# zenghjian/SceneSplat

Measured on AMD Instinct MI355X. Metric: Gaussians/s encoder fwd+bwd, 102k-pt chunks, higher is better.
Workload: dtype bf16

## Files before the change

include/scenesplat_hip.h:

```cpp
#ifndef SCENESPLAT_HIP_H
#define SCENESPLAT_HIP_H
#include <stddef.h>
#include <stdint.h>

#ifdef __cplusplus
extern "C" {
#endif

struct ihipStream_t;
typedef struct ihipStream_t* ss_stream_t;

#define SS_MAX_ORDERS 8
enum { SS_ORDER_Z = 0, SS_ORDER_Z_TRANS = 1, SS_ORDER_HILBERT = 2, SS_ORDER_HILBERT_TRANS = 3 };
enum { SS_DTYPE_F32 = 0, SS_DTYPE_BF16 = 1 };
enum { SS_ATTN_SIMT = 0, SS_ATTN_MFMA = 1 };
enum { SS_OK = 0, SS_ERR_ARG = 1, SS_ERR_LAUNCH = 2, SS_ERR_WORKSPACE = 3 };

int ss_version(void);

int ss_serialize_encode(const int32_t* grid_coord, const int32_t* batch, int64_t n, int depth, const int* orders,
                        int num_orders, int64_t* codes, ss_stream_t stream);
int ss_offsets_to_batch(const int32_t* offsets, int num_batches, int64_t n, int32_t* batch, ss_stream_t stream);
int ss_count_duplicates(const int64_t* sorted_keys, int64_t n, int32_t* count, ss_stream_t stream);
int ss_grid_coord_max(const int32_t* grid_coord, int64_t n, int32_t* out_max, ss_stream_t stream);
// ... 86 lines not shown

int ss_subm_conv_fwd(const void* in, const void* weight, const float* bias, const int32_t* nbr, const int32_t* rowperm,
                     void* out, int64_t n, int cin, int cout, int taps, int out_dtype, ss_stream_t stream);
int ss_subm_weight_mirror(const void* w, void* wt, int cout, int taps, int cin, ss_stream_t stream);
int ss_stream_create_cu_mask(int nwords, const uint32_t* mask, void** stream_out);
int ss_subm_im2col(const void* src, const int32_t* nbr, void* dst, int64_t n, int taps, int64_t row_bytes, ss_stream_t stream);
int ss_gemm8_ok(int64_t m, int k, int n, int taps);
int ss_subm_conv_fwd_pipe(const void* in, const void* weight, const float* bias, const int32_t* nbr, const int32_t* rowperm,
                          void* out, int64_t n, int cin, int cout, int taps, int out_dtype, ss_stream_t stream);
int ss_subm_conv_fwd_pipe_walk(const void* in, const void* weight, const float* bias, const int32_t* nbr_walk, const int32_t* rowperm,
                               void* out, int64_t n, int cin, int cout, int taps, int out_dtype, ss_stream_t stream);
int ss_subm_conv_fwd_uses_pipe(int64_t n, int cin, int cout, int taps);
int ss_subm_conv_fwd_walk(const void* in, const void* weight, const float* bias, const int32_t* nbr, const int32_t* nbr_walk,
                          const int32_t* rowperm, void* out, int64_t n, int cin, int cout, int taps, int out_dtype, ss_stream_t stream);
int ss_linear_fwd(const void* x, const void* weight, const float* bias, void* out, int64_t m, int k, int n, int out_dtype,
                  ss_stream_t stream);
int ss_wgrad_xcd_order(void);
int ss_wgrad_set_xcd_order(int on);
int ss_wgrad8_ok(int64_t n, int cin, int cout, int taps);
int ss_subm_conv_wgrad_pipe(const void* in, const void* dout, const int32_t* nbr, const int32_t* rowperm,
                            const int32_t* blk_count, const int32_t* blk_list, float* dweight, int64_t n, int cin, int cout,
                            int taps, ss_stream_t stream);
int ss_linear_wgrad(const void* x, const void* dy, float* dweight, float* dbias, int64_t m, int k_in, int n_out,
                    ss_stream_t stream);
int ss_linear_wgrad_group_plan(int64_t m, int k_in, int n_out, int64_t* desc_words);
int ss_linear_wgrad_tiles(int k_in, int n_out);
int ss_linear_wgrad_group_plan2(int64_t m, int k_in, int n_out, int launch_tiles, int64_t* desc_words);
int ss_linear_wgrad_group(const int64_t* desc, const int32_t* wg_start, int nprob, int total_workgroups, ss_stream_t stream);
int ss_linear_wgrad_group_plan_capped(int64_t m, int k_in, int n_out, int launch_tiles, int max_workgroups, int64_t* desc_words);
int ss_linear_wgrad_group_capped(const int64_t* desc, const int32_t* wg_start, int nprob, int total_items, int max_workgroups,
                                 ss_stream_t stream);
int ss_subm_conv_splits(int64_t n, int cout, int taps);
int ss_subm_conv_fwd_splitk(const void* in, const void* weight, const float* bias, const int32_t* nbr, const int32_t* rowperm,
                            float* acc32, int64_t n, int cin, int cout, int taps, int splits, ss_stream_t stream);
int ss_subm_block_lists(const int32_t* nbr, const int32_t* rowperm, int64_t n, int taps, int32_t* blk_count,
                        int32_t* blk_list, ss_stream_t stream);
int ss_subm_conv_wgrad(const void* in, const void* dout, const int32_t* nbr, const int32_t* rowperm,
                       const int32_t* blk_count, const int32_t* blk_list, float* dweight, int64_t n, int cin, int cout,
                       int taps, ss_stream_t stream);

int ss_subm_f32_ok(int cin_padded, int cout);
int ss_subm_f32_fwd(const float* in, const float* wq, const float* bias, const int32_t* nbr_walk, const int32_t* rowperm,
                    float* out, int64_t n, int cin_padded, int cout, int taps, ss_stream_t stream);
int ss_subm_f32_dgrad_dup(const float* dout_folded, const float* wq, const int32_t* nbr_walk, const int32_t* rowperm, float* din,
                          int64_t n, int cin_padded, int cout, int taps, ss_stream_t stream);
int ss_subm_f32_wgrad(const float* in, const float* dout, const int32_t* nbr_walk, const int32_t* rowperm,
                      const int32_t* blk_count, const int32_t* blk_list, float* dweight, int64_t n, int cin_padded,
                      int cin, int cout, int taps, ss_stream_t stream);

int ss_subm_conv_wgrad_pipe_walk(const void* in, const void* dout, const int32_t* nbr_walk, const int32_t* rowperm,
                                 const int32_t* blk_count, const int32_t* blk_list, float* dweight, int64_t n, int cin, int cout,
                                 int taps, ss_stream_t stream);
int ss_subm_conv_wgrad_uses_pipe(int64_t n, int cin, int cout, int taps);
int ss_subm_conv_wgrad_walk(const void* in, const void* dout, const int32_t* nbr, const int32_t* nbr_walk, const int32_t* rowperm,
                            const int32_t* blk_count, const int32_t* blk_list, float* dweight, int64_t n, int cin, int cout,
                            int taps, ss_stream_t stream);

int ss_add_layernorm_fwd(const void* x, int x_dtype, const void* y, int y_dtype, const float* rowscale,
                         const float* gamma, const float* beta, float eps, void* xout, int xout_dtype, void* xcopy_bf16,
                         void* h, int h_dtype, float* mean, float* rstd, int64_t n, int channels, ss_stream_t stream);
int ss_ln_add_ln_fwd(const void* x, int x_dtype, const void* t, int t_dtype, const float* gamma0, const float* beta0, float eps0,
                     const float* gamma1, const float* beta1, float eps1, float* xout, void* h, int h_dtype, float* stats,
                     int64_t n, int channels, ss_stream_t stream);
int ss_ln_add_ln_bwd(const float* g_xout, const void* g_h, int g_h_dtype, const float* xout, const void* t, int t_dtype,
                     const float* stats, const float* gamma0, const float* gamma1, void* g_x, int g_x_dtype, void* g_t,
                     int g_t_dtype, float* part, int64_t n, int channels, int nblocks, ss_stream_t stream);
int ss_add_layernorm_bwd_blocks(int64_t n);

int ss_block_tail_rows(void);
int ss_block_tail_bwd_blocks(int64_t n);
int ss_block_tail_fwd(const void* feat, const float* x, const float* rs1, const float* rs2, const void* wp, const void* bp,
                      const void* w1, const void* b1, const void* w2, const void* b2, int bias_dtype, const float* gamma, const float* beta,
                      float eps, float* x_mid, float* mean, float* rstd, void* h2, void* u, void* a, float* x_out,
                      void* xcopy_bf16, int64_t n, int channels, ss_stream_t stream);
int ss_block_tail_bwd(const float* g_xout, const void* g_xcopy_bf16, const float* x_mid, const float* mean, const float* rstd,
                      const void* u, const float* rs1, const float* rs2, const float* gamma, const void* wp_t, const void* w1_t,
                      const void* w2_t, float* g_mid, void* dfeat, void* dy2, void* du, void* dy1, float* part, int64_t n,
                      int channels, int nblocks, ss_stream_t stream);
int ss_group_partial_sums_outputs_per_workgroup(void);
int ss_group_partial_sums(const int64_t* desc, const int32_t* wg_start, int nprob, int total_workgroups, ss_stream_t stream);
int ss_transpose16_group(const int64_t* desc, const int32_t* wg_start, int nprob, int total_workgroups, ss_stream_t stream);
int ss_subm_weight_mirror_group_tile(void);
int ss_subm_weight_mirror_group(const int64_t* desc, const int32_t* wg_start, int nprob, int total_workgroups, ss_stream_t stream);
int ss_add_layernorm_bwd(const void* g_xout, int g_xout_dtype, const void* g_xcopy, int g_xcopy_dtype, const void* g_h,
                         int g_h_dtype, const void* v, int v_dtype, const float* mean, const float* rstd,
                         const float* gamma, const float* rowscale, void* g_x, int g_x_dtype, void* g_y, int g_y_dtype,
                         float* dgamma_part, float* dbeta_part, int64_t n, int channels, int nblocks, ss_stream_t stream);

int ss_col_stats(const void* x, int x_dtype, float* shift_out, float* psum, float* psq, int64_t n, int channels,
                 int nblocks, ss_stream_t stream);
int ss_bn_stats_finish(const float* part, const float* shift, int nblocks, int channels, int64_t n, float momentum, float eps,
                       float* running_mean, float* running_var, int64_t* num_batches, float* mean, float* rstd,
                       ss_stream_t stream);
int ss_bn_bwd_finish(const float* part, int nblocks, int channels, int64_t n, float* sums, float* coef, ss_stream_t stream);
int ss_bn_act_fwd(const void* x, int x_dtype, const float* mean, const float* rstd, const float* gamma, const float* beta,
                  int act, void* y, int y_dtype, int64_t n, int channels, ss_stream_t stream);
int ss_bn_act_bwd_reduce(const void* dy, int dy_dtype, const void* x, int x_dtype, const float* mean, const float* rstd,
                         const float* gamma, const float* beta, int act, float* pdz, float* pdzx, int64_t n, int channels,
                         int nblocks, ss_stream_t stream);
int ss_bn_act_bwd_apply(const void* dy, int dy_dtype, const void* x, int x_dtype, const float* mean, const float* rstd,
                        const float* gamma, const float* beta, int act, const float* c1, const float* c2, void* dx,
                        int dx_dtype, int64_t n, int channels, ss_stream_t stream);

int ss_feat_text_scan(const void* feat_bf16, const void* text_bf16, int64_t n, int dim, int num_classes, float* max_prob,
                      int32_t* argmax, const int32_t* idx, float* pred_accum, ss_stream_t stream);

// ... 208 lines not shown
```

scenesplat_amd/csrc/wgrad8.hip:

```cpp
#include "grouped.h"
#include <stdlib.h>

typedef __attribute__((ext_vector_type(8))) __bf16 w8_bf8_t;
typedef __attribute__((ext_vector_type(4))) short w8_s4_t;
typedef __attribute__((ext_vector_type(8))) short w8_s8_t;
typedef __attribute__((address_space(3))) w8_s4_t w8_lds_s4_t;
#define W8_MFMA(a, b, c) __builtin_amdgcn_mfma_f32_16x16x32_bf16((a), (b), (c), 0, 0, 0)

#define W8_BUF 65536
#define W8_HALF 16384
#define W8_OFF_B 32768
#define W8_CHUNK 60
#define W8_OFF_ISITE 131072
#define W8_OFF_JSITE (W8_OFF_ISITE + W8_CHUNK * 64 * 4)
#define W8_LDS_BYTES (W8_OFF_JSITE + W8_CHUNK * 64 * 4)
#define W8_ZERO_ELEMS 4096

__device__ uint4 w8_zero[W8_ZERO_ELEMS / 8];

__device__ __forceinline__ void w8_glds16(const void* gsrc, unsigned lds_wave_base) {
  asm volatile("s_mov_b32 m0, %1\n\ts_nop 0\n\tglobal_load_lds_dwordx4 %0, off" ::"v"(gsrc), "s"(lds_wave_base) : "memory");
}
__device__ __forceinline__ w8_bf8_t w8_tr2(const char* p) {
  w8_s4_t lo = __builtin_amdgcn_ds_read_tr16_b64_v4i16((w8_lds_s4_t*)(p));
// ... 255 lines not shown
  const int row = 8 * W8_XG, full = nb / row * row;
  if (L >= full) return L;
  const int xcd = L & 7, slot = L >> 3;
  return ((slot / W8_XG) * 8 + xcd) * W8_XG + slot % W8_XG;
}

template <bool GATHER>
__global__ void __launch_bounds__(512)
k_wgrad8(const unsigned short* __restrict__ X, const unsigned short* __restrict__ DY, const int32_t* __restrict__ nbr,
         const int32_t* __restrict__ rowperm, const int32_t* __restrict__ blk_count, const int32_t* __restrict__ blk_list,
         float* __restrict__ dW, float* __restrict__ dbias, int n, int Cin, int Cout, int taps, int ntn, int nblocks_total,
         int min_per, int ntiles, int nshares, int walk) {
  int L = (int)blockIdx.x;
  if (walk & 2) L = w8_xcd_order(L, (int)gridDim.x);
  w8_body<GATHER>(X, DY, nbr, rowperm, blk_count, blk_list, dW, dbias, n, Cin, Cout, taps, ntn, nblocks_total, min_per, ntiles,
                  nshares, L, walk & 1);
}

__global__ void __launch_bounds__(512)
k_wgrad8_group(const int64_t* __restrict__ desc, const int32_t* __restrict__ wg_start, int nprob, int nprob_flags) {
  const int b = blockIdx.x;
  const int p = group_owner(wg_start, nprob, b);
  const int64_t* d = desc + (int64_t)p * 8;
  const int64_t m = d[4];
  const uint64_t w5 = (uint64_t)d[5], w6 = (uint64_t)d[6], w7 = (uint64_t)d[7];
  const int k_in = (int)(w5 & 0xffffffffu), n_out = (int)(w5 >> 32);
  const int ntn = (int)(w6 & 0xffffffffu), ntiles = (int)(w6 >> 32);
  const int nshares = (int)(w7 & 0xffffffffu), min_per = (int)(w7 >> 32);
  int L = b - wg_start[p];
  if (nprob_flags & 1) {
    const int a = (8 - (wg_start[p] & 7)) & 7;
    if (L >= a) L = a + w8_xcd_order(L - a, nshares * ntiles - a);
  }
  w8_body<false>((const unsigned short*)d[0], (const unsigned short*)d[1], nullptr, nullptr, nullptr, nullptr, (float*)d[2],
                 (float*)d[3], (int)m, k_in, n_out, 1, ntn, (int)((m + 63) / 64), min_per, ntiles, nshares, L);
}

__global__ void __launch_bounds__(512)
k_wgrad8_group_capped(const int64_t* __restrict__ desc, const int32_t* __restrict__ wg_start, int nprob, int total_items) {
  for (int b = blockIdx.x; b < total_items; b += (int)gridDim.x) {
    const int p = group_owner(wg_start, nprob, b);
    const int64_t* d = desc + (int64_t)p * 8;
    const int64_t m = d[4];
    const uint64_t w5 = (uint64_t)d[5], w6 = (uint64_t)d[6], w7 = (uint64_t)d[7];
    const int k_in = (int)(w5 & 0xffffffffu), n_out = (int)(w5 >> 32);
    const int ntn = (int)(w6 & 0xffffffffu), ntiles = (int)(w6 >> 32);
    const int nshares = (int)(w7 & 0xffffffffu), min_per = (int)(w7 >> 32);
    w8_body<false>((const unsigned short*)d[0], (const unsigned short*)d[1], nullptr, nullptr, nullptr, nullptr, (float*)d[2],
                   (float*)d[3], (int)m, k_in, n_out, 1, ntn, (int)((m + 63) / 64), min_per, ntiles, nshares, b - wg_start[p]);
    __syncthreads();
  }
}

static int w8_xcd_flag = -1;
extern "C" int ss_wgrad_xcd_order(void) {
  if (w8_xcd_flag < 0) { const char* e = getenv("SS_WGRAD_XCD_TRIPLE"); w8_xcd_flag = (e && atoi(e) == 1) ? 1 : 0; }
  return w8_xcd_flag;
}
extern "C" int ss_wgrad_set_xcd_order(int on) { w8_xcd_flag = on ? 1 : 0; return SS_OK; }

extern "C" int ss_wgrad8_ok(int64_t n, int cin, int cout, int taps) {
  return n > 0 && n < (1LL << 31) && cin >= 8 && (cin & 7) == 0 && cin <= W8_ZERO_ELEMS && cout >= 8 && (cout & 7) == 0 &&
         cout <= W8_ZERO_ELEMS && taps >= 1;
}

static int w8_min_per(int64_t busy_tiles, int64_t est_blocks) {
  int64_t per = busy_tiles * est_blocks / 200;
  if (per < 8) per = 8;
  if (per > 160) per = 160;
  return (int)per;
}

static int w8_conv_launch(const void* in, const void* dout, const int32_t* nbr, const int32_t* rowperm, const int32_t* blk_count,
                          const int32_t* blk_list, float* dweight, int64_t n, int cin, int cout, int taps, int walk, hipStream_t stream);

extern "C" int ss_subm_conv_wgrad_pipe(const void* in, const void* dout, const int32_t* nbr, const int32_t* rowperm,
                                       const int32_t* blk_count, const int32_t* blk_list, float* dweight, int64_t n,
                                       int cin, int cout, int taps, hipStream_t stream) {
  return w8_conv_launch(in, dout, nbr, rowperm, blk_count, blk_list, dweight, n, cin, cout, taps, 0, stream);
}
extern "C" int ss_subm_conv_wgrad_pipe_walk(const void* in, const void* dout, const int32_t* nbr_walk, const int32_t* rowperm,
                                            const int32_t* blk_count, const int32_t* blk_list, float* dweight, int64_t n,
                                            int cin, int cout, int taps, hipStream_t stream) {
  return w8_conv_launch(in, dout, nbr_walk, rowperm, blk_count, blk_list, dweight, n, cin, cout, taps, 1, stream);
}

static int w8_conv_launch(const void* in, const void* dout, const int32_t* nbr, const int32_t* rowperm, const int32_t* blk_count,
                          const int32_t* blk_list, float* dweight, int64_t n, int cin, int cout, int taps, int walk, hipStream_t stream) {
  if (n == 0) return SS_OK;
  if (!ss_wgrad8_ok(n, cin, cout, taps) || !blk_count || !blk_list || !nbr) return SS_ERR_ARG;
  const int nblocks = ss_div_up(n, 64);
  const int tm = ss_div_up(cout, 256), tn = ss_div_up(cin, 256);
  static int env_per = -2;
  if (env_per == -2) { const char* e = getenv("SS_WGRAD_MINPER"); env_per = e ? atoi(e) : -1; }
  int min_per = env_per > 0 ? env_per : w8_min_per((int64_t)tm * tn * ((taps + 2) / 3), (int64_t)nblocks * 7 / 10);
  int splits = ss_div_up(nblocks, min_per);
  if (ss_wgrad_xcd_order()) walk |= 2;
  dim3 g((unsigned)((int64_t)taps * splits * tm * tn));
  SS_LAUNCH((k_wgrad8<true>), g, dim3(512), 0, stream, (const unsigned short*)in, (const unsigned short*)dout, nbr, rowperm,
            blk_count, blk_list, dweight, (float*)nullptr, (int)n, cin, cout, taps, tn, nblocks, min_per, tm * tn, splits, walk);
  return SS_OK;
}

static void w8_linear_plan(int64_t m, int k_in, int n_out, int* tm_, int* tn_, int* min_per_, int* splits_, int launch_tiles = 0) {
  const int nblocks = ss_div_up(m, 64);
  const int tm = ss_div_up(n_out, 256), tn = ss_div_up(k_in, 256);
  static int env_per = -2;
  if (env_per == -2) { const char* e = getenv("SS_WGRAD_MINPER"); env_per = e ? atoi(e) : -1; }
  static const int cus = [] {
    int dev = 0, n = 256;
    if (hipGetDevice(&dev) == hipSuccess) (void)hipDeviceGetAttribute(&n, hipDeviceAttributeMultiprocessorCount, dev);
    return n > 0 ? n : 256;
  }();
  const int tiles_all = launch_tiles > tm * tn ? launch_tiles : tm * tn;
  const int shares = cus / tiles_all > 0 ? cus / tiles_all : 1;
  int min_per = env_per > 0 ? env_per : (int)((nblocks + shares - 1) / shares);
  if (env_per <= 0 && min_per < 8) min_per = 8;
  if (min_per > nblocks) min_per = nblocks;
  *tm_ = tm; *tn_ = tn; *min_per_ = min_per; *splits_ = ss_div_up(nblocks, min_per);
}

extern "C" int ss_linear_wgrad_tiles(int k_in, int n_out) { return ss_div_up(n_out, 256) * ss_div_up(k_in, 256); }
extern "C" int ss_linear_wgrad_group_plan2(int64_t m, int k_in, int n_out, int launch_tiles, int64_t* desc_words) {
  if (m <= 0 || !ss_wgrad8_ok(m, k_in, n_out, 1) || !desc_words) return 0;
  int tm, tn, min_per, splits;
  w8_linear_plan(m, k_in, n_out, &tm, &tn, &min_per, &splits, launch_tiles);
  desc_words[5] = (int64_t)((uint64_t)(uint32_t)k_in | ((uint64_t)(uint32_t)n_out << 32));
  desc_words[6] = (int64_t)((uint64_t)(uint32_t)tn | ((uint64_t)(uint32_t)(tm * tn) << 32));
  desc_words[7] = (int64_t)((uint64_t)(uint32_t)splits | ((uint64_t)(uint32_t)min_per << 32));
  return splits * tm * tn;
}
extern "C" int ss_linear_wgrad_group_plan(int64_t m, int k_in, int n_out, int64_t* desc_words) {
  return ss_linear_wgrad_group_plan2(m, k_in, n_out, 0, desc_words);
}

#define W8_CAP_ROUNDS 4
extern "C" int ss_linear_wgrad_group_plan_capped(int64_t m, int k_in, int n_out, int launch_tiles, int max_workgroups,
                                                 int64_t* desc_words) {
  if (m <= 0 || max_workgroups <= 0 || !ss_wgrad8_ok(m, k_in, n_out, 1) || !desc_words) return 0;
  const int nblocks = ss_div_up(m, 64);
  const int tm = ss_div_up(n_out, 256), tn = ss_div_up(k_in, 256);
  const int64_t tiles_all = launch_tiles > tm * tn ? launch_tiles : tm * tn;
  int64_t shares = (int64_t)W8_CAP_ROUNDS * max_workgroups / tiles_all;
  if (shares < 1) shares = 1;
  if (shares > nblocks / 8) shares = nblocks / 8 > 0 ? nblocks / 8 : 1;
  int min_per = nblocks, splits = 1;
  for (int s = (int)shares; s > 1; --s) {
    const int per = ss_div_up(nblocks, s), n = ss_div_up(nblocks, per);
// ... 39 lines not shown
```

scenesplat_amd/functional.py:

```python
import os
import weakref

import torch
from torch.utils.weak import WeakIdKeyDictionary

from . import native as nv


def _bf16_autocast(x=None):
    return (x is None or x.is_cuda) and torch.is_autocast_enabled() and torch.get_autocast_dtype("cuda") == torch.bfloat16


class _WindowAttention(torch.autograd.Function):
    @staticmethod
    def forward(ctx, qkv, win, num_heads, scale, impl):
        qkv = qkv.contiguous()
        out, lse = nv.window_attn_fwd(qkv, win, num_heads, scale, impl)
        ctx.save_for_backward(qkv, out, lse)
        ctx.win, ctx.num_heads, ctx.scale, ctx.impl = win, num_heads, scale, impl
        return out

    @staticmethod
    def backward(ctx, dout):
        qkv, out, lse = ctx.saved_tensors
# ... 111 lines not shown
        if ctx.needs_input_grad[0]:
            dx = torch.zeros_like(x)
            if not ctx.has_dup:
                buf = torch.empty_like(g)
                for t in range(taps):
                    nv.gather_rows(g, nbr[t], out=buf)
                    dx.addmm_(buf, w[:, taps - 1 - t, :])
            else:
                for t in range(taps):
                    rows = torch.nonzero(nbr[t] >= 0, as_tuple=True)[0]
                    if rows.numel():
                        dx.index_add_(0, nbr[t][rows].long(), g[rows] @ w[:, t, :])
            dx = dx.to(ctx.in_dtype)
        if ctx.needs_input_grad[1]:
            dw = torch.empty((taps, cout, x.shape[1]), dtype=cd, device=x.device)
            buf = torch.empty_like(x)
            gt = g.t()
            for t in range(taps):
                nv.gather_rows(x, nbr[t], out=buf)
                torch.mm(gt, buf, out=dw[t])
            dw = dw.permute(1, 0, 2).reshape(weight.shape).to(weight.dtype)
        if ctx.has_bias and ctx.needs_input_grad[2]:
            db = g.sum(0).to(weight.dtype)
        return dx, dw, db, None, None, None, None


def _conv_meta(feat, weight, bias):
    return feat.dtype, weight.dtype, weight.shape, weight.shape[-1], bias is not None


def _pad8(x, w):
    pad = (-x.shape[1]) % 8
    if pad:
        x = torch.nn.functional.pad(x, (0, pad)); w = torch.nn.functional.pad(w, (0, pad))
    return x, w, pad


def _dup_fold(dup_fn, nbr, g):
    runs = dup_fn() if dup_fn is not None else nv.dup_runs_from_rulebook(nbr)
    return runs, nv.dup_fold_rows(g, runs)


def _conv_blocks(blocks_fn, nbr, rowperm):
    return blocks_fn() if blocks_fn is not None else nv.subm_block_lists(nbr, rowperm)


def _bias_grad(g, w_dtype):
    return g.sum(0, dtype=torch.float32).to(w_dtype)


class _SubMConv3dFused(torch.autograd.Function):

    @staticmethod
    def forward(ctx, feat, weight, bias, nbr, rowperm, blocks_fn, has_dup, walk_fn=None, dup_fn=None):
        taps, n = nbr.shape
        cout, cin = weight.shape[0], weight.shape[-1]
        x, w, pad = _pad8(feat.to(torch.bfloat16), bf16_of(weight).reshape(cout, taps, cin))
        x, w = x.contiguous(), w.contiguous()
        ctx.meta = _conv_meta(feat, weight, bias)
        ctx.blocks_fn, ctx.has_dup, ctx.dup_fn = blocks_fn, has_dup, dup_fn
        ctx.wt = mirrored_of(weight) if not pad else None
        ctx.im2col = n <= CONV_IM2COL_MAX_SITES
        out_dtype = torch.bfloat16 if torch.is_autocast_enabled() else torch.float32
        if ctx.im2col:
            cols = nv.subm_im2col(x, nbr)
            out = torch.nn.functional.linear(cols, w.view(cout, -1), bf16_of(bias))
            ctx.save_for_backward(cols, w, nbr, rowperm)
            return out.to(out_dtype)
        walk = None
        if CONV_WALK_RULEBOOK and walk_fn is not None and rowperm is not None and nv.subm_conv_fwd_uses_pipe(n, cin + pad, cout, taps):
            walk = walk_fn()
        ctx.has_walk = walk is not None
        out = nv.subm_conv_fwd(x, w, None if bias is None else bias.float().contiguous(), nbr, rowperm, out_dtype, nbr_walk=walk)
        ctx.save_for_backward(x, w, nbr, rowperm, *(() if walk is None else (walk,)))
        return out

    @staticmethod
    def backward(ctx, dout):
        x, w, nbr, rowperm = ctx.saved_tensors[:4]
        walk = ctx.saved_tensors[4] if getattr(ctx, "has_walk", False) else None
        in_dtype, w_dtype, w_shape, cin, has_bias = ctx.meta
        g = dout.to(torch.bfloat16).contiguous()
        dx = dw = db = None
        if ctx.needs_input_grad[0]:
            runs, gd = _dup_fold(ctx.dup_fn, nbr, g) if ctx.has_dup else (None, g)
            wt = ctx.wt if ctx.wt is not None else nv.subm_weight_mirror(w)
            if ctx.im2col:
                dx = torch.nn.functional.linear(nv.subm_im2col(gd, nbr), wt.view(wt.shape[0], -1))
            else:
                dx = nv.subm_conv_fwd(gd, wt, None, nbr, rowperm, nbr_walk=walk)
            if runs is not None:
                nv.dup_zero_rows_(dx, runs)
            dx = dx[:, :cin].to(in_dtype)
        if ctx.needs_input_grad[1]:
            if ctx.im2col:
                dw = _mm_f32(g.t(), x).view(w.shape)
            else:
                dw = nv.subm_conv_wgrad(x, g, nbr, rowperm, _conv_blocks(ctx.blocks_fn, nbr, rowperm), nbr_walk=walk)
            dw = dw[:, :, :cin].reshape(w_shape).to(w_dtype)
        if has_bias and ctx.needs_input_grad[2]:
            db = _bias_grad(g, w_dtype)
        return dx, dw, db, None, None, None, None, None, None


def _split_bf16(t):
    t = t.float()
    hi = t.to(torch.bfloat16)
    return hi, (t - hi.float()).to(torch.bfloat16)


class _SubMConv3dSplit(torch.autograd.Function):

    @staticmethod
    def forward(ctx, feat, weight, bias, nbr, rowperm, blocks_fn, has_dup=False, dup_fn=None):
        taps, n = nbr.shape
        cout, cin = weight.shape[0], weight.shape[-1]
        ctx.has_dup, ctx.dup_fn = has_dup, dup_fn
        x, w, _ = _pad8(feat.float(), weight.float().reshape(cout, taps, cin))
        xh, xl = _split_bf16(x)
        wh, wl = _split_bf16(w)
        x3 = torch.cat([xh, xl, xh], 1).contiguous()
        w3 = torch.cat([wh, wh, wl], 2).contiguous()
        out = nv.subm_conv_fwd(x3, w3, None if bias is None else bias.float().contiguous(), nbr, rowperm, torch.float32)
        ctx.save_for_backward(xh, xl, wh, wl, nbr, rowperm)
        ctx.meta = _conv_meta(feat, weight, bias)
        ctx.blocks_fn = blocks_fn
        return out

    @staticmethod
    def backward(ctx, dout):
        xh, xl, wh, wl, nbr, rowperm = ctx.saved_tensors
        in_dtype, w_dtype, w_shape, cin, has_bias = ctx.meta
        gh, gl = _split_bf16(dout.contiguous())
        dx = dw = db = None
        if ctx.needs_input_grad[0]:
            wt3 = torch.cat([nv.subm_weight_mirror(wh), nv.subm_weight_mirror(wh), nv.subm_weight_mirror(wl)], 2).contiguous()
            runs = None
            fh, fl = gh, gl
            if ctx.has_dup:
                runs, folded = _dup_fold(ctx.dup_fn, nbr, dout.float().contiguous())
                fh, fl = _split_bf16(folded)
            g3 = torch.cat([fh, fl, fh], 1).contiguous()
            dx = nv.subm_conv_fwd(g3, wt3, None, nbr, rowperm, torch.float32)
            if runs is not None:
                nv.dup_zero_rows_(dx, runs)
            dx = dx[:, :cin].to(in_dtype)
        if ctx.needs_input_grad[1]:
            blocks = _conv_blocks(ctx.blocks_fn, nbr, rowperm)
            cp = xh.shape[1]
            d2 = nv.subm_conv_wgrad(torch.cat([xh, xl], 1).contiguous(), gh, nbr, rowperm, blocks)
            d1 = nv.subm_conv_wgrad(xh, gl, nbr, rowperm, blocks)
            dw = (d2[:, :, :cp] + d2[:, :, cp:] + d1)[:, :, :cin].reshape(w_shape).to(w_dtype)
        if has_bias and ctx.needs_input_grad[2]:
            db = _bias_grad(dout, w_dtype)
        return dx, dw, db, None, None, None, None, None
# ... 3 lines not shown

    @staticmethod
    def forward(ctx, feat, weight, bias, nbr, rowperm, blocks_fn, walk_fn, has_dup=False, dup_fn=None):
        taps, n = nbr.shape
        cout, cin = weight.shape[0], weight.shape[-1]
        cp = 16 if cin <= 16 else 32
        ctx.has_dup, ctx.dup_fn, ctx.plain_nbr = has_dup, dup_fn, nbr
        ctx.orig_nbr = nbr if blocks_fn is None else None
        nbr = walk_fn() if walk_fn is not None else nv.subm_walk_rulebook(nbr, rowperm)
        x = feat.float()
        if cp != cin:
            x = torch.nn.functional.pad(x, (0, cp - cin))
        x = x.contiguous()
        w = weight.float().reshape(cout, taps, cin)
        out = nv.subm_f32_fwd(x, nv.subm_f32_weight_layout(w), None if bias is None else bias.float().contiguous(), nbr, rowperm)
        ctx.save_for_backward(x, w, nbr, rowperm)
        ctx.meta = _conv_meta(feat, weight, bias)
        ctx.blocks_fn = blocks_fn
        return out

    @staticmethod
    def backward(ctx, dout):
        x, w, nbr, rowperm = ctx.saved_tensors
        in_dtype, w_dtype, w_shape, cin, has_bias = ctx.meta
        g = dout.float().contiguous()
        dx = dw = db = None
        if ctx.needs_input_grad[0]:
            gd = _dup_fold(ctx.dup_fn, ctx.plain_nbr, g)[1] if ctx.has_dup else g
            dx = nv.subm_f32_fwd(gd, nv.subm_f32_weight_layout(w, mirror=True), None, nbr, rowperm,
                                 winners_only=ctx.has_dup).to(in_dtype)
        if ctx.needs_input_grad[1]:
            blocks = _conv_blocks(ctx.blocks_fn, ctx.orig_nbr, rowperm)
            dw = nv.subm_f32_wgrad(x, g, nbr, rowperm, blocks, cin).reshape(w_shape).to(w_dtype)
        if has_bias and ctx.needs_input_grad[2]:
            db = _bias_grad(g, w_dtype)
        return dx, dw, db, None, None, None, None, None, None


CONV_WALK_RULEBOOK = os.environ.get("SS_CONV_WALK", "1") != "0"
CONV_F32_MFMA = os.environ.get("SS_CONV_F32_MFMA", "1") != "0"
CONV_IM2COL_MAX_SITES = int(os.environ.get("SS_CONV_IM2COL_MAX", "8192"))


def _mm_f32(a, b):
    try:
        return torch.mm(a, b, out_dtype=torch.float32)
    except (RuntimeError, NotImplementedError, TypeError):
        return torch.mm(a, b).float()


def subm_conv3d(feat, weight, bias, nbr, has_dup=False, compute_dtype=torch.float32, rowperm=None, blocks_fn=None, walk_fn=None,
                dup_fn=None):
    if compute_dtype == torch.bfloat16 and weight.shape[0] % 8 == 0:
        return _SubMConv3dFused.apply(feat, weight, bias, nbr, rowperm, blocks_fn, has_dup, walk_fn, dup_fn)
    if compute_dtype == "bf16x3":
        if (CONV_F32_MFMA and weight.shape[0] == 32 and weight.shape[-1] <= 32 and feat.is_cuda
                and (weight.shape[-1] == 32 or not feat.requires_grad)):
            return _SubMConv3dF32.apply(feat, weight, bias, nbr, rowperm, blocks_fn, walk_fn, has_dup, dup_fn)
        if weight.shape[0] % 8 == 0 and feat.is_cuda:
            return _SubMConv3dSplit.apply(feat, weight, bias, nbr, rowperm, blocks_fn, has_dup, dup_fn)
        compute_dtype = torch.float32
    return _SubMConv3d.apply(feat, weight, bias, nbr, has_dup, compute_dtype)


class _Gelu(torch.autograd.Function):

    @staticmethod
    def forward(ctx, x):
        x = x.contiguous()
        ctx.save_for_backward(x)
        return nv.gelu(x)

    @staticmethod
    def backward(ctx, dy):
        (x,) = ctx.saved_tensors
        dy = dy.contiguous().to(x.dtype)
        if not _aligned16(dy):
            dy = dy.clone()
        return nv.gelu(x, dy)


GELU_HIP = os.environ.get("SS_GELU_HIP", "1") != "0"


def _aligned16(t):
    return t.data_ptr() % 16 == 0 and t.storage_offset() * t.element_size() % 16 == 0


def gelu(x):
    if GELU_HIP and x.is_cuda and x.dtype in (torch.float32, torch.bfloat16) and _aligned16(x):
        return _Gelu.apply(x)
    return torch.nn.functional.gelu(x)


def lang_head_release():
    _HEAD_CACHE.clear()


class _LangHead(torch.autograd.Function):

    @staticmethod
    def forward(ctx, feat, target, mask, normalize, want_p):
        feat = feat.contiguous()
        if target is not None:
            target = target.contiguous()
            if target.dtype not in (torch.float32, torch.bfloat16):
                target = target.float()
# ... 121 lines not shown

def register_mirrored(weights):
    for p in weights:
        ent = _SHADOW.get(p)
        if ent is not None and p.dim() == 5 and p.shape[-1] % 8 == 0:
            cout, cin = p.shape[0], p.shape[-1]
            ent.want("m", (cin, p.numel() // (cout * cin), cout), p.device)


def register_transposed(weights):
    for p in weights:
        ent = _SHADOW.get(p)
        if ent is not None and p.dim() == 2:
            ent.want("t", (p.shape[1], p.shape[0]), p.device)


def unregister_transposed(weights):
    for ent in filter(None, map(_SHADOW.get, weights)):
        ent.set("t", None)


def unregister_mirrored(weights):
    for ent in filter(None, map(_SHADOW.get, weights)):
        ent.set("m", None)


def mirrored_of(p):
    ent = _current(p)
    return ent.m if ent is not None else None


def bf16_t_of(p):
    ent = _current(p)
    return ent.t if ent is not None else None


def bf16_of(p):
    if p is None or p.dtype == torch.bfloat16:
        return p
    ent = _current(p)
    return ent.bf16 if ent is not None else p.to(torch.bfloat16)


WGRAD_GROUP_MAX_ROWS = int(os.environ.get("SS_WGRAD_GROUP_MAX", str(1 << 22)))
_STAGE = {"cur": None, "route": {}}
_UNFLUSHED = set()


WGRAD_GROUP_MAX_BYTES = int(float(os.environ.get("SS_WGRAD_GROUP_MAX_GIB", "8")) * (1 << 30))


WGRAD_OVERLAP = os.environ.get("SS_WGRAD_OVERLAP", "1") != "0"
WGRAD_DEFER_MIN_ROWS = int(os.environ.get("SS_WGRAD_DEFER_MIN_ROWS", "16384"))
WGRAD_OVERLAP_FREE_CUS = int(os.environ.get("SS_WGRAD_OVERLAP_FREE_CUS", "80"))
_OVERLAP = {"armed": False, "stages": [], "items": [], "pairs": [], "held": [], "flight": None, "callback": False, "streams": {}}
OVERLAP_STATS = {"deferred": 0, "launched": 0, "joined": 0}


def wgrad_overlap_arm(on):
    if _OVERLAP["flight"] is not None or _OVERLAP["items"] or _OVERLAP["held"]:
        _overlap_clear()
    _OVERLAP["armed"] = bool(on) and WGRAD_OVERLAP and WGRAD_DEFER_MIN_ROWS > 0
    _OVERLAP["stages"] = []


def _overlap_clear():
    flight = _OVERLAP["flight"]
    if flight is not None and not torch.cuda.is_current_stream_capturing():
        flight[0].wait_stream(flight[1])
    _OVERLAP.update(armed=False, stages=[], items=[], pairs=[], held=[], flight=None, callback=False)


def _overlap_alias(stage, q):
    q = [(x, dy, dw.detach(), db.detach() if db is not None else None) for x, dy, dw, db in q]
    stage.late = stage.late or {}
    stage.late.update({t.data_ptr(): t for _, _, dw, db in q for t in (dw, db) if t is not None})
    if not _OVERLAP["callback"]:
        _OVERLAP["callback"] = True
        torch.autograd.Variable._execution_engine.queue_callback(_overlap_finish)
    return q


def _overlap_launch():
    items, _OVERLAP["items"] = _OVERLAP["items"], []
    main = torch.cuda.current_stream()
    dev = items[0][0].device
    side = _OVERLAP["streams"].get(dev)
    if side is None:
        side = _OVERLAP["streams"][dev] = torch.cuda.Stream(dev)
    side.wait_stream(main)
    cus = torch.cuda.get_device_properties(dev).multi_processor_count
    nv.linear_wgrad_group(items, max_workgroups=max(1, cus - WGRAD_OVERLAP_FREE_CUS), stream=side)
    _OVERLAP["flight"] = (main, side, items)
    OVERLAP_STATS["launched"] += 1


def _overlap_join():
    flight, _OVERLAP["flight"] = _OVERLAP["flight"], None
    held, _OVERLAP["held"] = _OVERLAP["held"], []
    if flight is None:
        return None
    main = flight[0]
    with torch.cuda.stream(main):
        main.wait_stream(flight[1])
        for stage, q in held:
            nv.linear_wgrad_group(q)
            stage.late = None
    OVERLAP_STATS["joined"] += 1
    return main


def _overlap_finish():
    try:
        cur = torch.cuda.current_stream()
        if _OVERLAP["items"]:
            items, _OVERLAP["items"] = _OVERLAP["items"], []
            nv.linear_wgrad_group(items)
        main = _overlap_join() or cur
        if cur != main:
            cur.wait_stream(main)
        for p, g in _OVERLAP["pairs"]:
            if p.grad is None or p.grad.data_ptr() != g.data_ptr():
                raise RuntimeError("a deferred weight gradient was copied before it was computed (a gradient hook?): "
                                   "run with SS_WGRAD_OVERLAP=0")
    finally:
        _overlap_clear()


class _WgradStage:
    def __init__(self, n_rows=0, params=()):
        self.queue = []
        self.redq = []
        self.bytes = 0
        self.n_rows = n_rows
        self.params = params
        self.defer = False
        self.prev = None
        self.late = None
        self.flushed = False
        self.hooked = True

    def add(self, x, dy, dw, db):
        self.queue.append((x, dy, dw, db))
        self.bytes += x.numel() * x.element_size() + dy.numel() * dy.element_size()
        if self.bytes > WGRAD_GROUP_MAX_BYTES:
            q, self.queue, self.bytes = self.queue, [], 0
            nv.linear_wgrad_group(q)

    def flush(self):
        _UNFLUSHED.discard(self)
        q, self.queue, self.bytes = self.queue, [], 0
        r, self.redq = self.redq, []
        first, self.flushed = not self.flushed, True
        flight = _OVERLAP["flight"] is not None
        late_ok = (q and (self.defer or flight) and not self.hooked and not torch.is_grad_enabled()
                   and all(p.grad is None for p in self.params))
        if late_ok and self.defer and not flight:
            _OVERLAP["items"] += _overlap_alias(self, q)
            OVERLAP_STATS["deferred"] += 1
            if self.prev is None or not self.prev.defer:
                _overlap_launch()
        elif late_ok:
            _OVERLAP["held"].append((self, _overlap_alias(self, q)))
        else:
            nv.linear_wgrad_group(q)
        if flight and first and (self.prev is None or max(self.n_rows, self.prev.n_rows) >= WGRAD_DEFER_MIN_ROWS):
            _overlap_join()
        nv.group_partial_sums(r)


class _StageParams(torch.autograd.Function):
    @staticmethod
    def forward(ctx, stage, *params):
        ctx.stage = stage
        ctx.set_materialize_grads(False)
        return tuple(p.view_as(p) for p in params)

    @staticmethod
    def backward(ctx, *grads):
        stage = ctx.stage
        stage.flush()
        ptrs, stage.late = stage.late, None
        if ptrs:
            _OVERLAP["pairs"] += [(p, ptrs[g.data_ptr()]) for p, g in zip(stage.params, grads) if g is not None and g.data_ptr() in ptrs]
        return (None,) + grads


def _overlap_enter(stage, hooked):
    stages = _OVERLAP["stages"]
    stage.defer = (bool(stage.params) and stage.n_rows >= WGRAD_DEFER_MIN_ROWS and not hooked
                   and any(st.n_rows < WGRAD_DEFER_MIN_ROWS for st in stages))
    stage.hooked = hooked
    stage.prev = stages[-1] if stages else None
    stages.append(stage)


def stage_begin(linears, n_rows):
    _STAGE["cur"], _STAGE["route"] = None, {}
    params = []
    if WGRAD_GROUP_MAX_ROWS and LINEAR_WGRAD_MIN_ROWS <= n_rows <= WGRAD_GROUP_MAX_ROWS and torch.is_grad_enabled() and _bf16_autocast():
        params = [p for m in linears for p in (m.weight, m.bias) if p is not None and p.requires_grad and p.dtype == torch.float32 and p.is_cuda]
    if not params:
        if _OVERLAP["armed"]:
            _overlap_enter(_WgradStage(n_rows), False)
        return
    stage = _WgradStage(n_rows, params)
    if _OVERLAP["armed"]:
        _overlap_enter(stage, any(getattr(p, "_post_accumulate_grad_hooks", None) or p._backward_hooks for p in params) or (
            torch.distributed.is_available() and torch.distributed.is_initialized() and torch.distributed.get_world_size() > 1))
    aliases = _StageParams.apply(stage, *params)
    _STAGE["cur"], _STAGE["route"] = stage, {id(p): a for p, a in zip(params, aliases)}


def stage_end():
    _STAGE["cur"], _STAGE["route"] = None, {}


def reset_state():
    stage_end()
# ... 531 lines not shown
```

scenesplat_amd/native.py:

```python
import ctypes

import numpy as np
import torch

from . import _lib, grouped
from ._lib import check

_C = _lib.CONSTANTS
F32, BF16 = _C["SS_DTYPE_F32"], _C["SS_DTYPE_BF16"]
ATTN_SIMT, ATTN_MFMA = _C["SS_ATTN_SIMT"], _C["SS_ATTN_MFMA"]
HAVE_MFMA_ATTN = True
ORDER_IDS = {name: _C["SS_ORDER_" + name.upper().replace("-", "_")] for name in ("z", "z-trans", "hilbert", "hilbert-trans")}


def _p(t):
    return ctypes.c_void_p(t.data_ptr()) if t is not None else ctypes.c_void_p(0)


def _stream():
    return ctypes.c_void_p(torch.cuda.current_stream().cuda_stream)


def _req(t, dtype=None, name="tensor", shape=None):
    if not isinstance(t, torch.Tensor) or not t.is_cuda:
# ... 209 lines not shown

def linear_fwd(x, w, bias=None, out_dtype=torch.bfloat16):
    m, k = x.shape
    n = w.shape[0]
    out = torch.empty((m, n), dtype=out_dtype, device=x.device)
    check(lib().ss_linear_fwd(_p(x), _p(w), _p(bias), _p(out), m, k, n, dtype_code(out), _stream()), "ss_linear_fwd")
    return out


def subm_block_lists(nbr, rowperm):
    taps, n = nbr.shape
    _req(nbr, torch.int32, "nbr")
    if rowperm is not None:
        _req(rowperm, torch.int32, "rowperm", (n,))
    nb = (n + 63) // 64
    cnt = torch.empty(taps, dtype=torch.int32, device=nbr.device)
    lst = torch.empty((taps, nb), dtype=torch.int32, device=nbr.device)
    check(lib().ss_subm_block_lists(_p(nbr), _p(rowperm), n, taps, _p(cnt), _p(lst), _stream()), "ss_subm_block_lists")
    return cnt, lst


_ARENA = {"buf": None, "off": 0}


def zero_arena_begin(numel, device):
    _ARENA["buf"] = torch.zeros(int(numel), dtype=torch.float32, device=device) if numel > 0 else None
    _ARENA["off"] = 0


def zeros_f32(numel, device):
    buf, off = _ARENA["buf"], _ARENA["off"]
    if buf is not None and buf.device == device and off + numel <= buf.numel():
        _ARENA["off"] = off + ((numel + 3) & ~3)
        return buf[off:off + numel]
    return torch.zeros(int(numel), dtype=torch.float32, device=device)


def subm_conv_wgrad(x, dout, nbr, rowperm, blocks, out=None, nbr_walk=None):
    n, cin = x.shape
    cout = dout.shape[1]
    taps = nbr.shape[0]
    _req(x, torch.bfloat16, "x"); _req(dout, torch.bfloat16, "dout", (n, cout)); _req(nbr, torch.int32, "nbr", (taps, n))
    if cin % 8 or cout % 8:
        raise RuntimeError("subm_conv_wgrad: channels must be multiples of 8")
    if rowperm is not None:
        _req(rowperm, torch.int32, "rowperm", (n,))
    dw = zeros_f32(cout * taps * cin, x.device).view(cout, taps, cin) if out is None else _req(out, torch.float32, "out", (cout, taps, cin))
    cnt, lst = blocks
    _req(cnt, torch.int32, "blk_count", (taps,)); _req(lst, torch.int32, "blk_list", (taps, (n + 63) // 64))
    if nbr_walk is not None:
        _req(nbr_walk, torch.int32, "nbr_walk", (taps, n))
    check(lib().ss_subm_conv_wgrad_walk(_p(x), _p(dout), _p(nbr), _p(nbr_walk), _p(rowperm), _p(cnt), _p(lst), _p(dw), n, cin, cout, taps,
                                        _stream()), "ss_subm_conv_wgrad_walk")
    return dw


def subm_f32_weight_layout(w, mirror=False):
    w = w.float()
    if mirror:
        w = w.flip(1).permute(2, 1, 0)
    co, taps, c = w.shape
    cp = 16 if c <= 16 else 32
    if co != 32 or c > 32:
        raise RuntimeError("subm_f32: 32 output channels, at most 32 input channels")
    if cp != c:
        w = torch.nn.functional.pad(w, (0, cp - c))
    return w.reshape(32, taps, cp // 8, 2, 4).permute(1, 2, 3, 0, 4).contiguous()


def subm_walk_rulebook(nbr, rowperm):
    return nbr if rowperm is None else nbr.index_select(1, rowperm).contiguous()


def subm_f32_fwd(x, wq, bias, nbr, rowperm, winners_only=False):
    n, cp = x.shape
    taps = nbr.shape[0]
    _req(x, torch.float32, "x"); _req(wq, torch.float32, "wq", (taps, cp // 8, 2, 32, 4)); _req(nbr, torch.int32, "nbr", (taps, n))
    if bias is not None:
        _req(bias, torch.float32, "bias", (32,))
    if rowperm is not None:
        _req(rowperm, torch.int32, "rowperm", (n,))
    out = torch.empty((n, 32), dtype=torch.float32, device=x.device)
    if winners_only:
        if bias is not None:
            raise RuntimeError("subm_f32_fwd: the dgrad form takes no bias")
        check(lib().ss_subm_f32_dgrad_dup(_p(x), _p(wq), _p(nbr), _p(rowperm), _p(out), n, cp, 32, taps, _stream()), "ss_subm_f32_dgrad_dup")
        return out
    check(lib().ss_subm_f32_fwd(_p(x), _p(wq), _p(bias), _p(nbr), _p(rowperm), _p(out), n, cp, 32, taps, _stream()), "ss_subm_f32_fwd")
    return out


def dup_runs_from_rulebook(nbr):
    keys, order = torch.sort(nbr[nbr.shape[0] // 2].long(), stable=True)
    return keys.contiguous(), order.to(torch.int32).contiguous()


def dup_fold_rows(src, runs):
    keys, order = runs
    n, C = src.shape
    _req(src, None, "src"); _req(keys, torch.int64, "sorted_keys", (n,)); _req(order, torch.int32, "order", (n,))
    out = torch.empty_like(src)
    check(lib().ss_dup_fold_rows(_p(src), _p(keys), _p(order), _p(out), n, C, dtype_code(src), _stream()), "ss_dup_fold_rows")
    return out


def dup_zero_rows_(x, runs):
# ... 1614 lines not shown
```

Measured before the change: 2.970 million.

## Defer sparse-conv weight gradients to a side stream with a capped persistent kernel

```diff
diff --git a/include/scenesplat_hip.h b/include/scenesplat_hip.h
--- a/include/scenesplat_hip.h
+++ b/include/scenesplat_hip.h
@@ -162,6 +162,10 @@
                                  const int32_t* blk_count, const int32_t* blk_list, float* dweight, int64_t n, int cin, int cout,
                                  int taps, ss_stream_t stream);
 int ss_subm_conv_wgrad_uses_pipe(int64_t n, int cin, int cout, int taps);
+int ss_subm_conv_wgrad_pipe_capped(const void* in, const void* dout, const int32_t* nbr, const int32_t* rowperm,
+                                   const int32_t* blk_count, const int32_t* blk_list, float* dweight, int32_t* counter, int64_t n,
+                                   int cin, int cout, int taps, int walk, int min_per, int max_workgroups, ss_stream_t stream);
+int64_t ss_subm_conv_wgrad_pipe_items(int64_t n, int cin, int cout, int taps, int min_per);
 int ss_subm_conv_wgrad_walk(const void* in, const void* dout, const int32_t* nbr, const int32_t* nbr_walk, const int32_t* rowperm,
                             const int32_t* blk_count, const int32_t* blk_list, float* dweight, int64_t n, int cin, int cout,
                             int taps, ss_stream_t stream);
diff --git a/scenesplat_amd/csrc/wgrad8.hip b/scenesplat_amd/csrc/wgrad8.hip
--- a/scenesplat_amd/csrc/wgrad8.hip
+++ b/scenesplat_amd/csrc/wgrad8.hip
@@ -331,6 +331,23 @@
   }
 }
 
+__global__ void __launch_bounds__(512)
+k_wgrad8_conv_capped(const unsigned short* __restrict__ X, const unsigned short* __restrict__ DY, const int32_t* __restrict__ nbr,
+                     const int32_t* __restrict__ rowperm, const int32_t* __restrict__ blk_count,
+                     const int32_t* __restrict__ blk_list, float* __restrict__ dW, int32_t* __restrict__ counter, int n, int Cin,
+                     int Cout, int taps, int ntn, int nblocks_total, int min_per, int ntiles, int nshares, int walk, int total_items) {
+  __shared__ int ticket;
+  for (;;) {
+    if (threadIdx.x == 0) ticket = atomicAdd(counter, 1);
+    __syncthreads();
+    const int L = ticket;
+    __syncthreads();
+    if (L >= total_items) break;
+    w8_body<true>(X, DY, nbr, rowperm, blk_count, blk_list, dW, nullptr, n, Cin, Cout, taps, ntn, nblocks_total, min_per, ntiles,
+                  nshares, L, walk);
+  }
+}
+
 static int w8_xcd_flag = -1;
 extern "C" int ss_wgrad_xcd_order(void) {
   if (w8_xcd_flag < 0) { const char* e = getenv("SS_WGRAD_XCD_TRIPLE"); w8_xcd_flag = (e && atoi(e) == 1) ? 1 : 0; }
@@ -350,8 +367,43 @@
   return (int)per;
 }
 
+static int w8_conv_min_per(int nblocks, int tiles, int taps) {
+  static int env_per = -2;
+  if (env_per == -2) { const char* e = getenv("SS_WGRAD_MINPER"); env_per = e ? atoi(e) : -1; }
+  return env_per > 0 ? env_per : w8_min_per((int64_t)tiles * ((taps + 2) / 3), (int64_t)nblocks * 7 / 10);
+}
+
 static int w8_conv_launch(const void* in, const void* dout, const int32_t* nbr, const int32_t* rowperm, const int32_t* blk_count,
                           const int32_t* blk_list, float* dweight, int64_t n, int cin, int cout, int taps, int walk, hipStream_t stream);
+
+extern "C" int ss_subm_conv_wgrad_pipe_capped(const void* in, const void* dout, const int32_t* nbr, const int32_t* rowperm,
+                                              const int32_t* blk_count, const int32_t* blk_list, float* dweight, int32_t* counter,
+                                              int64_t n, int cin, int cout, int taps, int walk, int min_per, int max_workgroups,
+                                              hipStream_t stream) {
+  if (n == 0) return SS_OK;
+  if (!ss_wgrad8_ok(n, cin, cout, taps) || !blk_count || !blk_list || !nbr || !counter || min_per < 0 || max_workgroups <= 0)
+    return SS_ERR_ARG;
+  const int nblocks = ss_div_up(n, 64);
+  const int tm = ss_div_up(cout, 256), tn = ss_div_up(cin, 256);
+  if (min_per == 0) min_per = w8_conv_min_per(nblocks, tm * tn, taps);
+  if (min_per > nblocks) min_per = nblocks;
+  const int splits = ss_div_up(nblocks, min_per);
+  const int64_t items = (int64_t)taps * splits * tm * tn;
+  if (items >= (1LL << 30)) return SS_ERR_ARG;
+  const int grid = items < max_workgroups ? (int)items : max_workgroups;
+  SS_LAUNCH(k_wgrad8_conv_capped, dim3((unsigned)grid), dim3(512), 0, stream, (const unsigned short*)in, (const unsigned short*)dout,
+            nbr, rowperm, blk_count, blk_list, dweight, counter, (int)n, cin, cout, taps, tn, nblocks, min_per, tm * tn, splits,
+            walk ? 1 : 0, (int)items);
+  return SS_OK;
+}
+extern "C" int64_t ss_subm_conv_wgrad_pipe_items(int64_t n, int cin, int cout, int taps, int min_per) {
+  if (n <= 0 || !ss_wgrad8_ok(n, cin, cout, taps) || min_per < 0) return 0;
+  const int nblocks = ss_div_up(n, 64);
+  const int tiles = ss_div_up(cout, 256) * ss_div_up(cin, 256);
+  if (min_per == 0) min_per = w8_conv_min_per(nblocks, tiles, taps);
+  if (min_per > nblocks) min_per = nblocks;
+  return (int64_t)taps * ss_div_up(nblocks, min_per) * tiles;
+}
 
 extern "C" int ss_subm_conv_wgrad_pipe(const void* in, const void* dout, const int32_t* nbr, const int32_t* rowperm,
                                        const int32_t* blk_count, const int32_t* blk_list, float* dweight, int64_t n,
@@ -370,9 +422,7 @@
   if (!ss_wgrad8_ok(n, cin, cout, taps) || !blk_count || !blk_list || !nbr) return SS_ERR_ARG;
   const int nblocks = ss_div_up(n, 64);
   const int tm = ss_div_up(cout, 256), tn = ss_div_up(cin, 256);
-  static int env_per = -2;
-  if (env_per == -2) { const char* e = getenv("SS_WGRAD_MINPER"); env_per = e ? atoi(e) : -1; }
-  int min_per = env_per > 0 ? env_per : w8_min_per((int64_t)tm * tn * ((taps + 2) / 3), (int64_t)nblocks * 7 / 10);
+  int min_per = w8_conv_min_per(nblocks, tm * tn, taps);
   int splits = ss_div_up(nblocks, min_per);
   if (ss_wgrad_xcd_order()) walk |= 2;
   dim3 g((unsigned)((int64_t)taps * splits * tm * tn));
diff --git a/scenesplat_amd/functional.py b/scenesplat_amd/functional.py
--- a/scenesplat_amd/functional.py
+++ b/scenesplat_amd/functional.py
@@ -187,13 +187,14 @@
 class _SubMConv3dFused(torch.autograd.Function):
 
     @staticmethod
-    def forward(ctx, feat, weight, bias, nbr, rowperm, blocks_fn, has_dup, walk_fn=None, dup_fn=None):
+    def forward(ctx, feat, weight, bias, nbr, rowperm, blocks_fn, has_dup, walk_fn=None, dup_fn=None, late=None):
         taps, n = nbr.shape
         cout, cin = weight.shape[0], weight.shape[-1]
         x, w, pad = _pad8(feat.to(torch.bfloat16), bf16_of(weight).reshape(cout, taps, cin))
         x, w = x.contiguous(), w.contiguous()
         ctx.meta = _conv_meta(feat, weight, bias)
         ctx.blocks_fn, ctx.has_dup, ctx.dup_fn = blocks_fn, has_dup, dup_fn
+        ctx.late = late if not pad else None
         ctx.wt = mirrored_of(weight) if not pad else None
         ctx.im2col = n <= CONV_IM2COL_MAX_SITES
         out_dtype = torch.bfloat16 if torch.is_autocast_enabled() else torch.float32
@@ -231,11 +232,16 @@
             if ctx.im2col:
                 dw = _mm_f32(g.t(), x).view(w.shape)
             else:
-                dw = nv.subm_conv_wgrad(x, g, nbr, rowperm, _conv_blocks(ctx.blocks_fn, nbr, rowperm), nbr_walk=walk)
+                blocks = _conv_blocks(ctx.blocks_fn, nbr, rowperm)
+                if _conv_wgrad_defers(getattr(ctx, "late", None), x, g, nbr.shape[0], w_dtype):
+                    dw = nv.zeros_f32(w.numel(), x.device).view(w.shape)
+                    _overlap_queue_conv(ctx.late[1], (x, g, nbr, rowperm, blocks, walk, dw.detach()))
+                else:
+                    dw = nv.subm_conv_wgrad(x, g, nbr, rowperm, blocks, nbr_walk=walk)
             dw = dw[:, :, :cin].reshape(w_shape).to(w_dtype)
         if has_bias and ctx.needs_input_grad[2]:
             db = _bias_grad(g, w_dtype)
-        return dx, dw, db, None, None, None, None, None, None
+        return dx, dw, db, None, None, None, None, None, None, None
 
 
 def _split_bf16(t):
@@ -345,7 +351,9 @@
 def subm_conv3d(feat, weight, bias, nbr, has_dup=False, compute_dtype=torch.float32, rowperm=None, blocks_fn=None, walk_fn=None,
                 dup_fn=None):
     if compute_dtype == torch.bfloat16 and weight.shape[0] % 8 == 0:
-        return _SubMConv3dFused.apply(feat, weight, bias, nbr, rowperm, blocks_fn, has_dup, walk_fn, dup_fn)
+        stage = _STAGE["cur"]
+        late = (stage, weight) if (CONV_WGRAD_OVERLAP and stage is not None and stage.defer) else None
+        return _SubMConv3dFused.apply(feat, weight, bias, nbr, rowperm, blocks_fn, has_dup, walk_fn, dup_fn, late)
     if compute_dtype == "bf16x3":
         if (CONV_F32_MFMA and weight.shape[0] == 32 and weight.shape[-1] <= 32 and feat.is_cuda
                 and (weight.shape[-1] == 32 or not feat.requires_grad)):
@@ -573,13 +581,26 @@
 
 WGRAD_OVERLAP = os.environ.get("SS_WGRAD_OVERLAP", "1") != "0"
 WGRAD_DEFER_MIN_ROWS = int(os.environ.get("SS_WGRAD_DEFER_MIN_ROWS", "16384"))
-WGRAD_OVERLAP_FREE_CUS = int(os.environ.get("SS_WGRAD_OVERLAP_FREE_CUS", "80"))
-_OVERLAP = {"armed": False, "stages": [], "items": [], "pairs": [], "held": [], "flight": None, "callback": False, "streams": {}}
+CONV_WGRAD_OVERLAP = os.environ.get("SS_CONV_WGRAD_OVERLAP", "1") != "0"
+WGRAD_OVERLAP_FREE_CUS = int(os.environ.get("SS_WGRAD_OVERLAP_FREE_CUS", "72" if CONV_WGRAD_OVERLAP else "80"))
+CONV_WGRAD_OVERLAP_MIN_PER = int(os.environ.get("SS_CONV_WGRAD_OVERLAP_MIN_PER", "0"))
+WGRAD_OVERLAP_JOIN = os.environ.get("SS_WGRAD_OVERLAP_JOIN", "end" if CONV_WGRAD_OVERLAP else "large")
+WGRAD_OVERLAP_START_SKIP = int(os.environ.get("SS_WGRAD_OVERLAP_START_SKIP", "0"))
+WGRAD_OVERLAP_HELD_SIDE = os.environ.get("SS_WGRAD_OVERLAP_HELD_SIDE", "0") == "1"
+_OVERLAP = {"armed": False, "stages": [], "items": [], "convs": [], "pairs": [], "held": [], "flight": None, "callback": False,
+            "skip": 0, "streams": {}}
 OVERLAP_STATS = {"deferred": 0, "launched": 0, "joined": 0}
+CONV_OVERLAP_STATS = {"deferred": 0, "capped": 0, "inline": 0}
+
+
+def overlap_join_due(mode, rows, next_rows, defers, next_defers, min_rows):
+    if mode == "end":
+        return bool(defers or next_defers)
+    return next_rows is None or max(rows, next_rows) >= min_rows
 
 
 def wgrad_overlap_arm(on):
-    if _OVERLAP["flight"] is not None or _OVERLAP["items"] or _OVERLAP["held"]:
+    if _OVERLAP["flight"] is not None or _OVERLAP["items"] or _OVERLAP["held"] or _OVERLAP["convs"]:
         _overlap_clear()
     _OVERLAP["armed"] = bool(on) and WGRAD_OVERLAP and WGRAD_DEFER_MIN_ROWS > 0
     _OVERLAP["stages"] = []
@@ -589,17 +610,41 @@
     flight = _OVERLAP["flight"]
     if flight is not None and not torch.cuda.is_current_stream_capturing():
         flight[0].wait_stream(flight[1])
-    _OVERLAP.update(armed=False, stages=[], items=[], pairs=[], held=[], flight=None, callback=False)
+    _OVERLAP.update(armed=False, stages=[], items=[], convs=[], pairs=[], held=[], flight=None, callback=False, skip=0)
 
 
 def _overlap_alias(stage, q):
     q = [(x, dy, dw.detach(), db.detach() if db is not None else None) for x, dy, dw, db in q]
     stage.late = stage.late or {}
     stage.late.update({t.data_ptr(): t for _, _, dw, db in q for t in (dw, db) if t is not None})
+    _overlap_callback()
+    return q
+
+
+def _overlap_callback():
     if not _OVERLAP["callback"]:
         _OVERLAP["callback"] = True
         torch.autograd.Variable._execution_engine.queue_callback(_overlap_finish)
-    return q
+
+
+def _conv_wgrad_defers(late, x, g, taps, w_dtype):
+    if late is None or not (CONV_WGRAD_OVERLAP and _OVERLAP["armed"]) or _OVERLAP["flight"] is not None:
+        return False
+    stage, p = late
+    if not stage.defer or stage.hooked or w_dtype != torch.float32 or p.grad is not None or torch.is_grad_enabled():
+        return False
+    if getattr(p, "_post_accumulate_grad_hooks", None) or p._backward_hooks:
+        return False
+    if torch.distributed.is_available() and torch.distributed.is_initialized() and torch.distributed.get_world_size() > 1:
+        return False
+    return bool(nv.lib().ss_subm_conv_wgrad_uses_pipe(x.shape[0], x.shape[1], g.shape[1], taps))
+
+
+def _overlap_queue_conv(p, item):
+    _OVERLAP["convs"].append(item)
+    _OVERLAP["pairs"].append((p, item[-1]))
+    CONV_OVERLAP_STATS["deferred"] += 1
+    _overlap_callback()
 
 
 def _overlap_launch():
@@ -611,8 +656,14 @@
         side = _OVERLAP["streams"][dev] = torch.cuda.Stream(dev)
     side.wait_stream(main)
     cus = torch.cuda.get_device_properties(dev).multi_processor_count
-    nv.linear_wgrad_group(items, max_workgroups=max(1, cus - WGRAD_OVERLAP_FREE_CUS), stream=side)
-    _OVERLAP["flight"] = (main, side, items)
+    cap = max(1, cus - WGRAD_OVERLAP_FREE_CUS)
+    nv.linear_wgrad_group(items, max_workgroups=cap, stream=side)
+    convs, _OVERLAP["convs"] = _OVERLAP["convs"], []
+    for x, g, nbr, rowperm, blocks, walk, dw in sorted(convs, key=lambda c: -c[0].shape[0] * c[0].shape[1] * c[1].shape[1]):
+        nv.subm_conv_wgrad_capped(x, g, nbr, rowperm, blocks, out=dw, nbr_walk=walk, max_workgroups=cap,
+                                  min_per=CONV_WGRAD_OVERLAP_MIN_PER, stream=side)
+        CONV_OVERLAP_STATS["capped"] += 1
+    _OVERLAP["flight"] = (main, side, [items, convs])
     OVERLAP_STATS["launched"] += 1
 
 
@@ -637,6 +688,10 @@
         if _OVERLAP["items"]:
             items, _OVERLAP["items"] = _OVERLAP["items"], []
             nv.linear_wgrad_group(items)
+        convs, _OVERLAP["convs"] = _OVERLAP["convs"], []
+        for x, g, nbr, rowperm, blocks, walk, dw in convs:
+            nv.subm_conv_wgrad(x, g, nbr, rowperm, blocks, out=dw, nbr_walk=walk)
+            CONV_OVERLAP_STATS["inline"] += 1
         main = _overlap_join() or cur
         if cur != main:
             cur.wait_stream(main)
@@ -680,12 +735,24 @@
             _OVERLAP["items"] += _overlap_alias(self, q)
             OVERLAP_STATS["deferred"] += 1
             if self.prev is None or not self.prev.defer:
-                _overlap_launch()
+                _OVERLAP["skip"] = WGRAD_OVERLAP_START_SKIP if self.prev is not None else 0
+                if not _OVERLAP["skip"]:
+                    _overlap_launch()
+        elif late_ok and WGRAD_OVERLAP_HELD_SIDE:
+            q = _overlap_alias(self, q)
+            _OVERLAP["flight"][1].wait_stream(torch.cuda.current_stream())
+            nv.linear_wgrad_group(q, stream=_OVERLAP["flight"][1])
+            _OVERLAP["flight"][2].append(q)
         elif late_ok:
             _OVERLAP["held"].append((self, _overlap_alias(self, q)))
         else:
             nv.linear_wgrad_group(q)
-        if flight and first and (self.prev is None or max(self.n_rows, self.prev.n_rows) >= WGRAD_DEFER_MIN_ROWS):
+            if first and not flight and _OVERLAP["items"] and _OVERLAP["skip"] > 0:
+                _OVERLAP["skip"] -= 1
+                if not _OVERLAP["skip"] or self.prev is None or self.prev.defer:
+                    _overlap_launch()
+        if flight and first and overlap_join_due(WGRAD_OVERLAP_JOIN, self.n_rows, self.prev.n_rows if self.prev is not None else None,
+                                                 self.defer, self.prev is not None and self.prev.defer, WGRAD_DEFER_MIN_ROWS):
             _overlap_join()
         nv.group_partial_sums(r)
 
diff --git a/scenesplat_amd/native.py b/scenesplat_amd/native.py
--- a/scenesplat_amd/native.py
+++ b/scenesplat_amd/native.py
@@ -285,6 +285,31 @@
         _req(nbr_walk, torch.int32, "nbr_walk", (taps, n))
     check(lib().ss_subm_conv_wgrad_walk(_p(x), _p(dout), _p(nbr), _p(nbr_walk), _p(rowperm), _p(cnt), _p(lst), _p(dw), n, cin, cout, taps,
                                         _stream()), "ss_subm_conv_wgrad_walk")
+    return dw
+
+
+def subm_conv_wgrad_capped(x, dout, nbr, rowperm, blocks, out=None, nbr_walk=None, max_workgroups=None, min_per=0, stream=None):
+    if stream is not None:
+        with torch.cuda.stream(stream):
+            return subm_conv_wgrad_capped(x, dout, nbr, rowperm, blocks, out, nbr_walk, max_workgroups, min_per)
+    n, cin = x.shape
+    cout = dout.shape[1]
+    taps = nbr.shape[0]
+    _req(x, torch.bfloat16, "x"); _req(dout, torch.bfloat16, "dout", (n, cout)); _req(nbr, torch.int32, "nbr", (taps, n))
+    if rowperm is not None:
+        _req(rowperm, torch.int32, "rowperm", (n,))
+    cnt, lst = blocks
+    _req(cnt, torch.int32, "blk_count", (taps,)); _req(lst, torch.int32, "blk_list", (taps, (n + 63) // 64))
+    if nbr_walk is not None:
+        _req(nbr_walk, torch.int32, "nbr_walk", (taps, n))
+    if max_workgroups is None:
+        max_workgroups = torch.cuda.get_device_properties(x.device).multi_processor_count
+    dw = torch.zeros((cout, taps, cin), dtype=torch.float32, device=x.device) if out is None else _req(out, torch.float32, "out", (cout, taps, cin))
+    counter = torch.zeros(1, dtype=torch.int32, device=x.device)
+    rule = nbr if nbr_walk is None else nbr_walk
+    check(lib().ss_subm_conv_wgrad_pipe_capped(_p(x), _p(dout), _p(rule), _p(rowperm), _p(cnt), _p(lst), _p(dw), _p(counter), n, cin, cout,
+                                               taps, int(nbr_walk is not None), int(min_per), int(max_workgroups), _stream()),
+          "ss_subm_conv_wgrad_pipe_capped")
     return dw
 
 
```

New measurement: 3.056 million (median of 6 runs). +2.9%, better.
